# little-little-point-cloud-group/buildingSegment

Measured on AMD Instinct MI355X. Metric: Mpoints/s segmented (kNN+normal+label), higher is better.
Workload: dtype int32 coordinates / f64 normals; 1 GPU; urban_50m; points_per_gpu=50000000, k=16, max_nn=50, rg_mode=0, largest_plane=135921, seed_attempts=6951, fallback_queries=0, rg_rounds=25, validation_rejects=2, tie_rows=971975, parallelism=1 GPU, whole path

## Files before the change

buildingsegment_amd/csrc/bs_knn.hip:

```cpp
#include <algorithm>
#include <cmath>
#include <cstdio>
#include <cstdlib>
#include <type_traits>

#include "bs_common.h"
#include "bs_normal.h"

namespace bs {

namespace {

constexpr int BS_FAST_RINGS = 2;
constexpr int BS_GENERAL_RINGS = 6;

template <bool TILED>
using GridOf = std::conditional_t<TILED, TiledGridDev, GridDev>;

template <bool TILED>
__device__ inline uint64_t cell_key(uint32_t cx, uint32_t cy, uint32_t cz, uint64_t kbase)
{
  if constexpr (TILED)
    return kbase | morton_cell(cx, cy, cz);
  else
    return pack_cell(cx, cy, cz);
}

__device__ inline void tile_enter(TiledGridDev& g, int64_t s, uint64_t& kbase, int64_t& lo, int64_t& hi)
{
  const int32_t t = tile_of(g.tile_off, g.n_tiles, s);
  const TileDesc d = g.tiles[t];
#pragma unroll
  for (int a = 0; a < 3; a++) {
    g.mn[a] = d.mn[a];
    g.dim[a] = d.dim[a];
  }
  kbase = (uint64_t)t << g.mbits;
  lo = g.tile_off[t];
  hi = g.tile_off[t + 1];
}

template <bool TILED = false>
__device__ inline bool cell_lookup(const GridDev& g, uint32_t cx, uint32_t cy, uint32_t cz, int& start,
                                   int& end, uint64_t kbase = 0)
{
  const uint64_t k = cell_key<TILED>(cx, cy, cz, kbase);
  uint32_t h = hash_cell(k) & g.hmask;
  for (;;) {
    const int4 raw = *reinterpret_cast<const int4*>(&g.table[h]);
    const uint64_t ek = (uint64_t)(uint32_t)raw.x | ((uint64_t)(uint32_t)raw.y << 32);
    if (ek == k) {
      start = raw.z;
      end = raw.w;
      return true;
    }
    if (ek == ~0ull)
      return false;
    h = (h + 1) & g.hmask;
  }
}

__device__ inline bool guaranteed_radius(const GridDev& g, const int q[3], const int ci[3], int rho,
                                         uint64_t& R2)
{
  uint32_t R = 0xFFFFFFFFu;
  bool bounded = false;
#pragma unroll
  for (int a = 0; a < 3; a++) {
    if (ci[a] - rho > 0) {
      int lo = g.mn[a] + (ci[a] - rho) * g.cell;
      R = min(R, (uint32_t)(q[a] - lo + 1));
      bounded = true;
    }
    if (ci[a] + rho < g.dim[a] - 1) {
      int hi = g.mn[a] + (ci[a] + rho + 1) * g.cell - 1;
      R = min(R, (uint32_t)(hi + 1 - q[a]));
      bounded = true;
    }
  }
  R2 = (uint64_t)R * (uint64_t)R;
  return bounded;
}

__device__ inline void moments_add(Moments& m, int x, int y, int z)
{
  m.sx += x;
  m.sy += y;
  m.sz += z;
  m.sxx += (uint64_t)((int64_t)x * x);
  m.syy += (uint64_t)((int64_t)y * y);
  m.szz += (uint64_t)((int64_t)z * z);
  m.sxy += (int64_t)x * y;
  m.sxz += (int64_t)x * z;
  m.syz += (int64_t)y * z;
  m.n += 1;
}

template <int KC, bool TILED = false>
__global__ __launch_bounds__(256) void knn_fast_kernel(GridOf<TILED> g, int64_t q_begin, int64_t q_end, int K,
                                                       int max_nn, double r2, int32_t* __restrict__ neigh,
                                                       double* __restrict__ normals,
                                                       int32_t* __restrict__ fb_list,
                                                       int32_t* __restrict__ fb_count, uint64_t cert_r2,
                                                       unsigned long long* __restrict__ uncert,
                                                       int32_t* __restrict__ npos, unsigned long long* __restrict__ tie_rows)
{
  const int64_t s = xcd_logical_block() * (int64_t)blockDim.x + threadIdx.x;
  if (s >= g.n)
    return;
  const int32_t loc = g.slocal[s];
  if (loc < q_begin || loc >= q_end)
    return;
  uint64_t kbase = 0;
  if constexpr (TILED) {
    int64_t lo, hi;
    tile_enter(g, s, kbase, lo, hi);
  }
  uint64_t runner = ~0ull;
  const int4 P = g.spts[s];
  const int q[3] = {P.x, P.y, P.z};
  const int ci[3] = {(int)((uint32_t)(P.x - g.mn[0]) / (uint32_t)g.cell),
                     (int)((uint32_t)(P.y - g.mn[1]) / (uint32_t)g.cell),
                     (int)((uint32_t)(P.z - g.mn[2]) / (uint32_t)g.cell)};
  uint64_t best[KC];
  int bpos[KC];
#pragma unroll
  for (int j = 0; j < KC; j++) {
    best[j] = ~0ull;
    bpos[j] = 0;
  }
  Moments m = {};
  bool done = false;
  for (int rho = 0; rho <= BS_FAST_RINGS && !done; rho++) {
    for (int dz = -rho; dz <= rho; dz++) {
      const int cz = ci[2] + dz;
      if (cz < 0 || cz >= g.dim[2])
        continue;
      for (int dy = -rho; dy <= rho; dy++) {
        const int cy = ci[1] + dy;
        if (cy < 0 || cy >= g.dim[1])
          continue;
        const bool face = (dz == -rho || dz == rho || dy == -rho || dy == rho);
        const int step = face ? 1 : (rho > 0 ? 2 * rho : 1);
        for (int dx = -rho; dx <= rho; dx += step) {
          const int cx = ci[0] + dx;
          if (cx < 0 || cx >= g.dim[0])
            continue;
          int cs, ce;
          if (!cell_lookup<TILED>(g, (uint32_t)cx, (uint32_t)cy, (uint32_t)cz, cs, ce, kbase))
            continue;
          for (int t = cs; t < ce; t++) {
            const int4 c = g.spts[t];
            const int ex = c.x - q[0], ey = c.y - q[1], ez = c.z - q[2];
            const uint32_t d2 = (uint32_t)(ex * ex) + (uint32_t)(ey * ey) + (uint32_t)(ez * ez);
            uint64_t key = ((uint64_t)d2 << 32) | (uint32_t)c.w;
            if (key < best[KC - 1]) {
              int pay = t;
#pragma unroll
              for (int j = 0; j < KC; j++) {
                const bool lt = key < best[j];
                const uint64_t hi = lt ? best[j] : key;
                const int ph = lt ? bpos[j] : pay;
                best[j] = lt ? key : best[j];
                bpos[j] = lt ? pay : bpos[j];
                key = hi;
                pay = ph;
              }
            }
            runner = key < runner ? key : runner;
            if ((double)d2 < r2)
              moments_add(m, c.x, c.y, c.z);
          }
        }
      }
    }
    uint64_t R2;
    const bool bounded = guaranteed_radius(g, q, ci, rho, R2);
    if (!bounded) {
      done = true;
    } else {
      uint64_t kth = ~0ull;
#pragma unroll
      for (int j = 0; j < KC; j++)
        kth = (j == K - 1) ? best[j] : kth;
      const bool knn_ok = kth != ~0ull && (kth >> 32) < R2;
      const bool nrm_ok = (double)R2 >= r2;
      done = knn_ok && nrm_ok;
    }
  }
  uint64_t kth_final = ~0ull;
#pragma unroll
  for (int j = 0; j < KC; j++)
    kth_final = (j == K - 1) ? best[j] : kth_final;
  if (!done || m.n > max_nn || kth_final == ~0ull) {
    const int slot = atomicAdd(fb_count, 1);
    fb_list[slot] = (int32_t)s;
    return;
  }
  int32_t* row = neigh + (int64_t)(loc - q_begin) * K;
#pragma unroll
  for (int j = 0; j < KC; j++)
    if (j < K)
      row[j] = (int32_t)(uint32_t)best[j];
  if (npos) {
    int32_t* prow = npos + s * K;
#pragma unroll
    for (int j = 0; j < KC; j++)
      if (j < K)
        prow[j] = bpos[j];
  }
  if (normals) {
    const V3 nv = normal_from_moments(m);
    double* o = normals + 3 * (int64_t)(loc - q_begin);
    o[0] = nv.x;
    o[1] = nv.y;
    o[2] = nv.z;
    if (npos) {
      double* po = pnorm_of(npos, g.n, K) + 3 * s;
      po[0] = nv.x;
      po[1] = nv.y;
      po[2] = nv.z;
    }
  }
  if (cert_r2 && (kth_final >> 32) >= cert_r2)
    atomicAdd(uncert, 1ull);
  if (tie_rows) {
    bool tie = false;
    uint64_t next = runner;
#pragma unroll
    for (int j = 0; j + 1 < KC; j++) {
      tie = tie || (j + 1 < K && (best[j] >> 32) == (best[j + 1] >> 32));
      next = (j + 1 == K) ? best[j + 1] : next;
    }
    tie = tie || (next != ~0ull && (next >> 32) == (kth_final >> 32));
    if (tie)
      atomicAdd(tie_rows, 1ull);
  }
}

#ifndef BS_KNN_CAP4
#define BS_KNN_CAP4 0
#endif
constexpr int KBUF = 8;
#ifndef BS_KNN_PROBE_GROUP
#define BS_KNN_PROBE_GROUP 3
#endif
#ifdef BS_PROBE
__device__ unsigned long long g_knn_probe[8];
#endif

template <int KC, bool REL32, bool TILED = false, bool STREAM = false>
__global__ __launch_bounds__(256) __attribute__((amdgpu_waves_per_eu(KC == 16 && REL32 && BS_KNN_CAP4 ? 4 : (KC == 16 && REL32 && STREAM ? 3 : 2)))) void knn_fast2_kernel(GridOf<TILED> g, int64_t q_begin, int64_t q_end, int K,
                                                       int max_nn, double r2, uint32_t r2le, int32_t* __restrict__ neigh,
                                                       double* __restrict__ normals,
                                                       int32_t* __restrict__ fb_list,
                                                       int32_t* __restrict__ fb_count, uint64_t cert_r2,
                                                       unsigned long long* __restrict__ uncert,
                                                       int32_t* __restrict__ npos, unsigned long long* __restrict__ tie_rows)
{
  const int64_t s = xcd_logical_block() * (int64_t)blockDim.x + threadIdx.x;
  if (s >= g.n)
    return;
  const int32_t loc = g.slocal[s];
  if (loc < q_begin || loc >= q_end)
    return;
  uint64_t kbase = 0;
  if constexpr (TILED) {
    int64_t lo, hi;
    tile_enter(g, s, kbase, lo, hi);
  }
  uint64_t runner = ~0ull;
  const int4 P = g.spts[s];
  const int q[3] = {P.x, P.y, P.z};
  const int ci[3] = {(int)((uint32_t)(P.x - g.mn[0]) / (uint32_t)g.cell),
                     (int)((uint32_t)(P.y - g.mn[1]) / (uint32_t)g.cell),
                     (int)((uint32_t)(P.z - g.mn[2]) / (uint32_t)g.cell)};
  __shared__ uint32_t blo[KBUF][256], bhi[KBUF][256];
  __shared__ int bps[KBUF][256];
  __shared__ int srs[STREAM ? 9 : 1][STREAM ? 256 : 1], sre[STREAM ? 9 : 1][STREAM ? 256 : 1];
  int nbuf = 0;
  uint64_t best[KC];
  int bpos[KC];
#pragma unroll
  for (int j = 0; j < KC; j++) {
    best[j] = ~0ull;
    bpos[j] = 0;
  }
  Moments m = {};
  int rsx = 0, rsy = 0, rsz = 0, rsxx = 0, rsyy = 0, rszz = 0, rsxy = 0, rsxz = 0, rsyz = 0, rn = 0;
  bool done = false;
  auto flush = [&]() __attribute__((always_inline)) {
    uint64_t bk[KBUF];
    int bp[KBUF];
#pragma unroll
    for (int i = 0; i < KBUF; i++) {
      const bool have = i < nbuf;
      bk[i] = have ? (((uint64_t)bhi[i][threadIdx.x] << 32) | blo[i][threadIdx.x]) : ~0ull;
      bp[i] = have ? bps[i][threadIdx.x] : 0;
    }
    nbuf = 0;
#define BS_CE(ka, pa, kb, pb)            \
  do {                                   \
    const bool sw_ = (kb) < (ka);        \
    const uint64_t tk_ = (ka);           \
    const int tp_ = (pa);                \
    (ka) = sw_ ? (kb) : (ka);            \
    (pa) = sw_ ? (pb) : (pa);            \
    (kb) = sw_ ? tk_ : (kb);             \
    (pb) = sw_ ? tp_ : (pb);             \
  } while (0)
    constexpr int net[19][2] = {{0, 1}, {2, 3}, {4, 5}, {6, 7}, {0, 2}, {1, 3}, {4, 6}, {5, 7}, {1, 2}, {5, 6},
                                {0, 4}, {3, 7}, {1, 5}, {2, 6}, {1, 4}, {3, 6}, {2, 4}, {3, 5}, {3, 4}};
#pragma unroll
    for (int c = 0; c < 19; c++)
      BS_CE(bk[net[c][0]], bp[net[c][0]], bk[net[c][1]], bp[net[c][1]]);
#pragma unroll
    for (int i = 0; i < KBUF; i++)
      BS_CE(best[KC - KBUF + i], bpos[KC - KBUF + i], bk[KBUF - 1 - i], bp[KBUF - 1 - i]);
#pragma unroll
    for (int i = 0; i < KBUF; i++)
      runner = bk[i] < runner ? bk[i] : runner;
#pragma unroll
    for (int d = KC / 2; d >= 1; d >>= 1) {
#pragma unroll
      for (int i = 0; i < KC; i++)
        if ((i & d) == 0)
          BS_CE(best[i], bpos[i], best[i + d], bpos[i + d]);
    }
#undef BS_CE
  };
  auto cand_slot = [&](const int4 c, const int t, const bool real) __attribute__((always_inline)) {
    const int ex = c.x - q[0], ey = c.y - q[1], ez = c.z - q[2];
    const uint32_t d2 = (uint32_t)(ex * ex) + (uint32_t)(ey * ey) + (uint32_t)(ez * ez);
    const uint64_t key = ((uint64_t)d2 << 32) | (uint32_t)c.w;
    if (real && key < best[KC - 1]) {
      blo[nbuf][threadIdx.x] = (uint32_t)key;
      bhi[nbuf][threadIdx.x] = d2;
      bps[nbuf][threadIdx.x] = t;
      nbuf++;
    } else if (real) {
      runner = key < runner ? key : runner;
    }
    if (__ballot(nbuf == KBUF))
      flush();
    if (real && d2 <= r2le) {
      if constexpr (REL32) {
        rsx += ex;
        rsy += ey;
        rsz += ez;
        rsxx += __mul24(ex, ex);
        rsyy += __mul24(ey, ey);
        rszz += __mul24(ez, ez);
        rsxy += __mul24(ex, ey);
        rsxz += __mul24(ex, ez);
        rsyz += __mul24(ey, ez);
        rn += 1;
      } else {
        moments_add(m, c.x, c.y, c.z);
      }
    }
  };
#ifdef BS_PROBE
  int probe_exec = 0, probe_cand = 0;
#define BS_PROBE_BATCH()                                                         \
  do {                                                                           \
    if (rho <= 1 && (int)(threadIdx.x & 63) == __ffsll((long long)__ballot(1)) - 1) \
      probe_exec++;                                                              \
  } while (0)
#define BS_PROBE_CELL(cnt) \
  do {                     \
    if (rho <= 1)          \
      probe_cand += (cnt); \
  } while (0)
#else
#define BS_PROBE_BATCH() \
  do {                   \
  } while (0)
#define BS_PROBE_CELL(cnt) \
  do {                     \
  } while (0)
#endif
  for (int rho = 0; rho <= BS_FAST_RINGS && !done; rho++) {
    const bool streamed = STREAM && rho == 1;
    if (streamed) {
#pragma unroll 1
      for (int dz = -1; dz <= 1; dz++) {
        const int cz = ci[2] + dz;
        const bool zok = cz >= 0 && cz < g.dim[2];
        int cnt = 0;
        constexpr int GP = BS_KNN_PROBE_GROUP;
        static_assert(9 % GP == 0, "probe groups tile the slab");
#pragma unroll
        for (int u0 = 0; u0 < 9; u0 += GP) {
          int4 raw[GP];
          uint64_t ck[GP];
          uint32_t hh[GP];
          bool want[GP];
#pragma unroll
          for (int w = 0; w < GP; w++) {
            const int u = u0 + w;
            const int cy = ci[1] + u / 3 - 1, cx = ci[0] + u % 3 - 1;
            want[w] = zok && cy >= 0 && cy < g.dim[1] && cx >= 0 && cx < g.dim[0] && !(dz == 0 && u == 4);
            ck[w] = cell_key<TILED>((uint32_t)(want[w] ? cx : ci[0]), (uint32_t)(want[w] ? cy : ci[1]),
                                    (uint32_t)(want[w] ? cz : ci[2]), kbase);
            hh[w] = hash_cell(ck[w]) & g.hmask;
            raw[w] = *reinterpret_cast<const int4*>(&g.table[hh[w]]);
          }
#pragma unroll
          for (int w = 0; w < GP; w++) {
            int cs = 0, ce = 0;
            if (want[w]) {
              for (;;) {
                const uint64_t ek = (uint64_t)(uint32_t)raw[w].x | ((uint64_t)(uint32_t)raw[w].y << 32);
                if (ek == ck[w]) {
                  cs = raw[w].z;
                  ce = raw[w].w;
                  break;
                }
                if (ek == ~0ull)
                  break;
                hh[w] = (hh[w] + 1) & g.hmask;
                raw[w] = *reinterpret_cast<const int4*>(&g.table[hh[w]]);
              }
            }
            BS_PROBE_CELL(ce - cs);
            if (cs < ce) {
              srs[cnt][threadIdx.x] = cs;
              sre[cnt][threadIdx.x] = ce;
              cnt++;
            }
          }
        }
        int cur = 0;
        int t0 = cnt > 0 ? srs[0][threadIdx.x] : 0, e0 = cnt > 0 ? sre[0][threadIdx.x] : 0;
        int s1 = cnt > 1 ? srs[1][threadIdx.x] : 0, e1 = cnt > 1 ? sre[1][threadIdx.x] : 0;
        while (t0 < e0) {
          BS_PROBE_BATCH();
          const int rem = e0 - t0;
          int ta[4];
          bool rl[4];
          int4 cc[4];
#pragma unroll
          for (int v = 0; v < 4; v++) {
            const int t1 = s1 + (v - rem);
            rl[v] = v < rem || t1 < e1;
            ta[v] = v < rem ? t0 + v : t1;
            cc[v] = g.spts[rl[v] ? ta[v] : (int)s];
          }
#pragma unroll
          for (int v = 0; v < 4; v++)
            cand_slot(cc[v], ta[v], rl[v]);
          const bool pop1 = rem <= 4;
          t0 += pop1 ? 0 : 4;
          if (__ballot(pop1)) {
            const bool more1 = pop1 && cur + 2 < cnt;
            const int i2 = min(cur + 2, 8);
            const int s2 = more1 ? srs[i2][threadIdx.x] : 0, e2 = more1 ? sre[i2][threadIdx.x] : 0;
            t0 = pop1 ? s1 + (4 - rem) : t0;
            e0 = pop1 ? e1 : e0;
            s1 = pop1 ? s2 : s1;
            e1 = pop1 ? e2 : e1;
            cur += pop1 ? 1 : 0;
            const bool pop2 = pop1 && e0 != 0 && t0 >= e0;
            if (__ballot(pop2)) {
              const bool more2 = pop2 && cur + 2 < cnt;
              const int i3 = min(cur + 2, 8);
              const int s3 = more2 ? srs[i3][threadIdx.x] : 0, e3 = more2 ? sre[i3][threadIdx.x] : 0;
              t0 = pop2 ? s1 : t0;
              e0 = pop2 ? e1 : e0;
              s1 = pop2 ? s3 : s1;
              e1 = pop2 ? e3 : e1;
              cur += pop2 ? 1 : 0;
            }
          }
        }
      }
    }
    for (int dz = -rho; !streamed && dz <= rho; dz++) {
      const int cz = ci[2] + dz;
      if (cz < 0 || cz >= g.dim[2])
        continue;
      for (int dy = -rho; dy <= rho; dy++) {
        const int cy = ci[1] + dy;
        if (cy < 0 || cy >= g.dim[1])
          continue;
        const bool face = (dz == -rho || dz == rho || dy == -rho || dy == rho);
        const int step = face ? 1 : (rho > 0 ? 2 * rho : 1);
        for (int dx0 = -rho; dx0 <= rho; dx0 += 3 * step) {
          int4 raw[3];
          uint64_t ck[3];
          uint32_t hh[3];
          bool want[3];
#pragma unroll
          for (int u = 0; u < 3; u++) {
            const int dx = dx0 + u * step;
            const int cx = ci[0] + dx;
            want[u] = dx <= rho && cx >= 0 && cx < g.dim[0];
            ck[u] = cell_key<TILED>((uint32_t)(want[u] ? cx : ci[0]), (uint32_t)cy, (uint32_t)cz, kbase);
            hh[u] = hash_cell(ck[u]) & g.hmask;
            raw[u] = *reinterpret_cast<const int4*>(&g.table[hh[u]]);
          }
          int cs3[3], ce3[3];
#pragma unroll
          for (int u = 0; u < 3; u++) {
            cs3[u] = 0;
            ce3[u] = 0;
            if (!want[u])
              continue;
            for (;;) {
              const uint64_t ek = (uint64_t)(uint32_t)raw[u].x | ((uint64_t)(uint32_t)raw[u].y << 32);
              if (ek == ck[u]) {
                cs3[u] = raw[u].z;
                ce3[u] = raw[u].w;
                break;
              }
              if (ek == ~0ull)
                break;
              hh[u] = (hh[u] + 1) & g.hmask;
              raw[u] = *reinterpret_cast<const int4*>(&g.table[hh[u]]);
            }
          }
#pragma unroll 1
          for (int u = 0; u < 3; u++) {
            const int cs = u == 0 ? cs3[0] : (u == 1 ? cs3[1] : cs3[2]);
            const int ce = u == 0 ? ce3[0] : (u == 1 ? ce3[1] : ce3[2]);
            BS_PROBE_CELL(ce - cs);
            for (int t0 = cs; t0 < ce; t0 += 4) {
              BS_PROBE_BATCH();
              int4 cc[4];
#pragma unroll
              for (int v = 0; v < 4; v++)
                cc[v] = g.spts[t0 + v < ce ? t0 + v : ce - 1];
#pragma unroll
              for (int v = 0; v < 4; v++)
                cand_slot(cc[v], t0 + v, t0 + v < ce);
            }
          }
        }
      }
    }
    if (__ballot(nbuf > 0))
      flush();
    uint64_t R2;
    const bool bounded = guaranteed_radius(g, q, ci, rho, R2);
    if (!bounded) {
      done = true;
    } else {
      uint64_t kth = ~0ull;
#pragma unroll
      for (int j = 0; j < KC; j++)
        kth = (j == K - 1) ? best[j] : kth;
      const bool knn_ok = kth != ~0ull && (kth >> 32) < R2;
      const bool nrm_ok = (double)R2 >= r2;
      done = knn_ok && nrm_ok;
    }
  }
#undef BS_PROBE_BATCH
#undef BS_PROBE_CELL
#ifdef BS_PROBE
  {
    const unsigned long long act = __ballot(1);
    const int lane = threadIdx.x & 63;
    const int need = (probe_cand + 3) / 4;
    int ex_sum = probe_exec, nd_max = need, nd_sum = need, ln = 1;
    for (int o = 32; o > 0; o >>= 1) {
      const int a = __shfl_xor(ex_sum, o), b = __shfl_xor(nd_max, o), c = __shfl_xor(nd_sum, o), d = __shfl_xor(ln, o);
      const bool ok = (act >> (lane ^ o)) & 1;
      ex_sum += ok ? a : 0;
      nd_max = ok && b > nd_max ? b : nd_max;
      nd_sum += ok ? c : 0;
      ln += ok ? d : 0;
    }
    if (lane == __ffsll((long long)act) - 1) {
      atomicAdd(&g_knn_probe[0], (unsigned long long)ex_sum);
      atomicAdd(&g_knn_probe[1], (unsigned long long)nd_max);
      atomicAdd(&g_knn_probe[2], (unsigned long long)nd_sum);
      atomicAdd(&g_knn_probe[3], (unsigned long long)ln);
      atomicAdd(&g_knn_probe[4], 1ull);
    }
  }
#endif
  uint64_t kth_final = ~0ull;
#pragma unroll
  for (int j = 0; j < KC; j++)
    kth_final = (j == K - 1) ? best[j] : kth_final;
  if constexpr (REL32) {
    const int64_t n64 = rn, qx = q[0], qy = q[1], qz = q[2];
    m.n = rn;
    m.sx = n64 * qx + rsx;
    m.sy = n64 * qy + rsy;
    m.sz = n64 * qz + rsz;
    m.sxx = (uint64_t)(n64 * qx * qx + 2 * qx * rsx + rsxx);
    m.syy = (uint64_t)(n64 * qy * qy + 2 * qy * rsy + rsyy);
    m.szz = (uint64_t)(n64 * qz * qz + 2 * qz * rsz + rszz);
    m.sxy = n64 * qx * qy + qx * rsy + qy * rsx + rsxy;
    m.sxz = n64 * qx * qz + qx * rsz + qz * rsx + rsxz;
    m.syz = n64 * qy * qz + qy * rsz + qz * rsy + rsyz;
  }
  if (!done || m.n > max_nn || kth_final == ~0ull) {
    const int slot = atomicAdd(fb_count, 1);
    fb_list[slot] = (int32_t)s;
    return;
  }
  int32_t* row = neigh + (int64_t)(loc - q_begin) * K;
#pragma unroll
  for (int j = 0; j < KC; j++)
    if (j < K)
      row[j] = (int32_t)(uint32_t)best[j];
  if (npos) {
    int32_t* prow = npos + s * K;
#pragma unroll
    for (int j = 0; j < KC; j++)
      if (j < K)
        prow[j] = bpos[j];
  }
  if (normals) {
    const V3 nv = normal_from_moments(m);
    double* o = normals + 3 * (int64_t)(loc - q_begin);
    o[0] = nv.x;
    o[1] = nv.y;
    o[2] = nv.z;
    if (npos) {
      double* po = pnorm_of(npos, g.n, K) + 3 * s;
      po[0] = nv.x;
      po[1] = nv.y;
      po[2] = nv.z;
    }
  }
  if (cert_r2 && (kth_final >> 32) >= cert_r2)
    atomicAdd(uncert, 1ull);
  if (tie_rows) {
    bool tie = false;
    uint64_t next = runner;
#pragma unroll
    for (int j = 0; j + 1 < KC; j++) {
      tie = tie || (j + 1 < K && (best[j] >> 32) == (best[j + 1] >> 32));
      next = (j + 1 == K) ? best[j + 1] : next;
    }
    tie = tie || (next != ~0ull && (next >> 32) == (kth_final >> 32));
    if (tie)
      atomicAdd(tie_rows, 1ull);
  }
}


__device__ inline bool cand_less(uint64_t d2a, int32_t ia, uint64_t d2b, int32_t ib)
{
  return d2a < d2b || (d2a == d2b && ia < ib);
}

__device__ inline void list_insert(uint64_t* d2s, int32_t* idxs, int32_t* poss, int& cnt, int cap, uint64_t d2, int32_t idx,
                                   int32_t pos, uint64_t* out_d2 = nullptr)
{
  int c = cnt;
  if (c == cap) {
    if (!cand_less(d2, idx, d2s[cap - 1], idxs[cap - 1])) {
      if (out_d2 && d2 < *out_d2)
        *out_d2 = d2;
      return;
    }
    if (out_d2 && d2s[cap - 1] < *out_d2)
      *out_d2 = d2s[cap - 1];
    c = cap - 1;
  }
  int j = c;
  while (j > 0 && cand_less(d2, idx, d2s[j - 1], idxs[j - 1])) {
    d2s[j] = d2s[j - 1];
    idxs[j] = idxs[j - 1];
    poss[j] = poss[j - 1];
    j--;
  }
  d2s[j] = d2;
  idxs[j] = idx;
  poss[j] = pos;
  cnt = c + 1;
}

__device__ inline void hybrid_insert(uint64_t* d2s, int32_t* gids, int32_t* poss, int& cnt, int cap,
                                     uint64_t d2, int32_t gid, int32_t pos)
{
  int c = cnt;
  if (c == cap) {
    if (!cand_less(d2, gid, d2s[cap - 1], gids[cap - 1]))
      return;
    c = cap - 1;
  }
  int j = c;
  while (j > 0 && cand_less(d2, gid, d2s[j - 1], gids[j - 1])) {
    d2s[j] = d2s[j - 1];
    gids[j] = gids[j - 1];
    poss[j] = poss[j - 1];
    j--;
  }
  d2s[j] = d2;
  gids[j] = gid;
  poss[j] = pos;
  cnt = c + 1;
}

template <bool TILED = false>
__global__ __launch_bounds__(64) void knn_general_kernel(GridOf<TILED> g, int64_t q_begin, int K, int max_nn,
                                                         double r2, int32_t* __restrict__ neigh,
                                                         double* __restrict__ normals,
                                                         const int32_t* __restrict__ fb_list,
                                                         const int32_t* __restrict__ fb_count,
                                                         uint64_t cert_r2,
                                                         unsigned long long* __restrict__ uncert,
                                                         int32_t* __restrict__ npos, unsigned long long* __restrict__ tie_rows)
{
  const int total = *fb_count;
  for (int w = blockIdx.x * blockDim.x + threadIdx.x; w < total; w += gridDim.x * blockDim.x) {
    const int32_t s = fb_list[w];
    const int32_t loc = g.slocal[s];
    uint64_t kbase = 0;
    int64_t scan_lo = 0, scan_hi = g.n;
    if constexpr (TILED)
      tile_enter(g, s, kbase, scan_lo, scan_hi);
    const int4 P = g.spts[s];
    const int q[3] = {P.x, P.y, P.z};
    const int ci[3] = {(int)((uint32_t)(P.x - g.mn[0]) / (uint32_t)g.cell),
                       (int)((uint32_t)(P.y - g.mn[1]) / (uint32_t)g.cell),
                       (int)((uint32_t)(P.z - g.mn[2]) / (uint32_t)g.cell)};
    uint64_t kd2[32], md2[64];
    int32_t kidx[32], kpos[32], mgid[64], mpos[64];
    int kc = 0, mc = 0;
    uint64_t runner = ~0ull;
    bool done = false;
    for (int rho = 0; rho <= BS_GENERAL_RINGS && !done; rho++) {
      for (int dz = -rho; dz <= rho; dz++) {
        const int cz = ci[2] + dz;
        if (cz < 0 || cz >= g.dim[2])
          continue;
        for (int dy = -rho; dy <= rho; dy++) {
          const int cy = ci[1] + dy;
          if (cy < 0 || cy >= g.dim[1])
            continue;
          const bool face = (dz == -rho || dz == rho || dy == -rho || dy == rho);
          const int step = face ? 1 : (rho > 0 ? 2 * rho : 1);
          for (int dx = -rho; dx <= rho; dx += step) {
            const int cx = ci[0] + dx;
            if (cx < 0 || cx >= g.dim[0])
              continue;
            int cs, ce;
            if (!cell_lookup<TILED>(g, (uint32_t)cx, (uint32_t)cy, (uint32_t)cz, cs, ce, kbase))
              continue;
            for (int t = cs; t < ce; t++) {
              const int4 c = g.spts[t];
              const int64_t ex = (int64_t)c.x - q[0], ey = (int64_t)c.y - q[1], ez = (int64_t)c.z - q[2];
              const uint64_t d2 = (uint64_t)(ex * ex) + (uint64_t)(ey * ey) + (uint64_t)(ez * ez);
              list_insert(kd2, kidx, kpos, kc, K, d2, c.w, t, &runner);
              if ((double)d2 < r2)
                hybrid_insert(md2, mgid, mpos, mc, max_nn, d2, c.w, t);
            }
          }
        }
      }
      uint64_t R2;
      const bool bounded = guaranteed_radius(g, q, ci, rho, R2);
      if (!bounded)
        done = true;
      else
        done = (kc == K) && (kd2[K - 1] < R2) && ((double)R2 >= r2);
    }
    if (!done) {
      kc = 0;
      mc = 0;
      runner = ~0ull;
      for (int64_t t = scan_lo; t < scan_hi; t++) {
        const int4 c = g.spts[t];
        const int64_t ex = (int64_t)c.x - q[0], ey = (int64_t)c.y - q[1], ez = (int64_t)c.z - q[2];
        const uint64_t d2 = (uint64_t)(ex * ex) + (uint64_t)(ey * ey) + (uint64_t)(ez * ez);
        list_insert(kd2, kidx, kpos, kc, K, d2, c.w, (int32_t)t, &runner);
        if ((double)d2 < r2)
          hybrid_insert(md2, mgid, mpos, mc, max_nn, d2, c.w, (int32_t)t);
      }
    }
    int32_t* row = neigh + (int64_t)(loc - q_begin) * K;
    for (int j = 0; j < K; j++)
      row[j] = kidx[j];
    if (npos)
      for (int j = 0; j < K; j++)
        npos[(int64_t)s * K + j] = kpos[j];
    if (normals) {
      Moments m = {};
      for (int j = 0; j < mc; j++) {
        const int4 c = g.spts[mpos[j]];
        moments_add(m, c.x, c.y, c.z);
      }
      const V3 nv = normal_from_moments(m);
      double* o = normals + 3 * (int64_t)(loc - q_begin);
      o[0] = nv.x;
      o[1] = nv.y;
      o[2] = nv.z;
      if (npos) {
        double* po = pnorm_of(npos, g.n, K) + 3 * (int64_t)s;
        po[0] = nv.x;
        po[1] = nv.y;
        po[2] = nv.z;
      }
    }
    if (cert_r2 && kd2[K - 1] >= cert_r2)
      atomicAdd(uncert, 1ull);
    if (tie_rows) {
      bool tie = runner == kd2[K - 1];
      for (int j = 0; j + 1 < K; j++)
        tie = tie || kd2[j] == kd2[j + 1];
      if (tie)
        atomicAdd(tie_rows, 1ull);
    }
  }
}

constexpr int GCAP = 2048;

template <bool TILED = false>
__global__ __launch_bounds__(64) void knn_general_wave_kernel(GridOf<TILED> g, int64_t q_begin, int K, int max_nn, double r2,
                                                              int32_t* __restrict__ neigh, double* __restrict__ normals,
                                                              const int32_t* __restrict__ fb_list,
                                                              const int32_t* __restrict__ fb_count, uint64_t cert_r2,
                                                              unsigned long long* __restrict__ uncert,
                                                              int32_t* __restrict__ npos, unsigned long long* __restrict__ tie_rows,
                                                              int32_t* __restrict__ fb2_list, int32_t* __restrict__ fb2_count)
{
  __shared__ uint64_t bd2[GCAP];
  __shared__ int32_t bidx[GCAP], bpos[GCAP];
  __shared__ int cxyz[64][3];
  const int lane = threadIdx.x;
  const int total = *fb_count;
  for (int w = blockIdx.x; w < total; w += gridDim.x) {
    const int32_t s = fb_list[w];
    const int32_t loc = g.slocal[s];
    uint64_t kbase = 0;
    if constexpr (TILED) {
      int64_t lo, hi;
      tile_enter(g, s, kbase, lo, hi);
    }
    const int4 P = g.spts[s];
    const int q[3] = {P.x, P.y, P.z};
    const int ci[3] = {(int)((uint32_t)(P.x - g.mn[0]) / (uint32_t)g.cell),
                       (int)((uint32_t)(P.y - g.mn[1]) / (uint32_t)g.cell),
                       (int)((uint32_t)(P.z - g.mn[2]) / (uint32_t)g.cell)};
    int count = 0;
    bool done = false, overflow = false;
    for (int rho = 0; rho <= BS_GENERAL_RINGS && !done && !overflow; rho++) {
      const int side = 2 * rho + 1, ncell = side * side * side;
      for (int c0 = 0; c0 < ncell; c0 += 64) {
        const int c = c0 + lane;
        const int dz = c / (side * side) - rho, dy = (c / side) % side - rho, dx = c % side - rho;
        const int cx = ci[0] + dx, cy = ci[1] + dy, cz = ci[2] + dz;
        const int cheb = max(max(abs(dx), abs(dy)), abs(dz));
        int cs = 0, ce = 0;
        if (c < ncell && cheb == rho && cx >= 0 && cx < g.dim[0] && cy >= 0 && cy < g.dim[1] && cz >= 0 && cz < g.dim[2]) {
          if (!cell_lookup<TILED>(g, (uint32_t)cx, (uint32_t)cy, (uint32_t)cz, cs, ce, kbase))
            cs = ce = 0;
        }
        for (int t = cs; __ballot(t < ce) != 0; t++) {
          const bool have = t < ce;
          const unsigned long long m = __ballot(have);
          const int slot = count + __popcll(m & ((1ull << lane) - 1ull));
          if (have && slot < GCAP) {
            const int4 p = g.spts[t];
            const int64_t ex = (int64_t)p.x - q[0], ey = (int64_t)p.y - q[1], ez = (int64_t)p.z - q[2];
            bd2[slot] = (uint64_t)(ex * ex) + (uint64_t)(ey * ey) + (uint64_t)(ez * ez);
            bidx[slot] = p.w;
            bpos[slot] = t;
          }
          count += __popcll(m);
        }
      }
      if (count > GCAP) {
        overflow = true;
        break;
      }
      int P2 = 64;
      while (P2 < count)
        P2 <<= 1;
      for (int i = count + lane; i < P2; i += 64) {
        bd2[i] = ~0ull;
        bidx[i] = 0x7fffffff;
        bpos[i] = 0;
      }
      __syncthreads();
      for (int k2 = 2; k2 <= P2; k2 <<= 1) {
        for (int j = k2 >> 1; j > 0; j >>= 1) {
          for (int i = lane; i < P2; i += 64) {
            const int l = i ^ j;
            if (l > i) {
              const uint64_t da = bd2[i], db = bd2[l];
              const int32_t ia = bidx[i], ib = bidx[l];
              const bool a_gt_b = da > db || (da == db && ia > ib);
              const bool up = (i & k2) == 0;
              if (a_gt_b == up) {
                bd2[i] = db;
                bd2[l] = da;
                bidx[i] = ib;
                bidx[l] = ia;
                const int32_t pa = bpos[i];
                bpos[i] = bpos[l];
                bpos[l] = pa;
              }
            }
          }
          __syncthreads();
        }
      }
      uint64_t R2;
      const bool bounded = guaranteed_radius(g, q, ci, rho, R2);
      if (!bounded)
        done = true;
      else
        done = count >= K && bd2[K - 1] < R2 && (double)R2 >= r2;
      __syncthreads();
    }
    if (overflow || !done || count < K) {
      if (lane == 0)
        fb2_list[atomicAdd(fb2_count, 1)] = s;
      __syncthreads();
      continue;
    }
    if (lane < K) {
      neigh[(int64_t)(loc - q_begin) * K + lane] = bidx[lane];
      if (npos)
        npos[(int64_t)s * K + lane] = bpos[lane];
    }
    if (normals) {
      const bool in = lane < max_nn && lane < count && (double)bd2[lane] < r2;
      const int mc = __popcll(__ballot(in));
      if (in) {
        const int4 p = g.spts[bpos[lane]];
        cxyz[lane][0] = p.x;
        cxyz[lane][1] = p.y;
        cxyz[lane][2] = p.z;
      }
      __syncthreads();
      if (lane == 0) {
        Moments m = {};
        for (int j = 0; j < mc; j++)
          moments_add(m, cxyz[j][0], cxyz[j][1], cxyz[j][2]);
        const V3 nv = normal_from_moments(m);
        double* o = normals + 3 * (int64_t)(loc - q_begin);
        o[0] = nv.x;
        o[1] = nv.y;
        o[2] = nv.z;
        if (npos) {
          double* po = pnorm_of(npos, g.n, K) + 3 * (int64_t)s;
          po[0] = nv.x;
          po[1] = nv.y;
          po[2] = nv.z;
        }
      }
    }
    if (lane == 0) {
      if (cert_r2 && bd2[K - 1] >= cert_r2)
        atomicAdd(uncert, 1ull);
      if (tie_rows) {
        bool tie = count > K && bd2[K] == bd2[K - 1];
        for (int j = 0; j + 1 < K; j++)
          tie = tie || bd2[j] == bd2[j + 1];
        if (tie)
          atomicAdd(tie_rows, 1ull);
      }
    }
    __syncthreads();
  }
}

__global__ void mark_all_kernel(GridDev g, int64_t q_begin, int64_t q_end, int32_t* fb_list,
                                int32_t* fb_count)
{
  const int64_t s = blockIdx.x * (int64_t)blockDim.x + threadIdx.x;
  if (s >= g.n)
    return;
  const int32_t loc = g.slocal[s];
  if (loc < q_begin || loc >= q_end)
    return;
  fb_list[atomicAdd(fb_count, 1)] = (int32_t)s;
}

}

template <bool TILED>
static int launch_knn(bs_ctx* ctx, const GridOf<TILED>& g, int64_t q_begin, int64_t q_end, const bs_params& p,
                      int32_t* d_neigh, double* d_normals, double cert_radius, int64_t* n_uncertified, int32_t* d_npos)
{
  hipStream_t st = ctx->stream;
  const int64_t n = g.n;
  BS_HIP(ctx, ctx->fb_list.reserve(sizeof(int32_t) * (2 * n + 32)));
  int32_t* fb_list = ctx->fb_list.as<int32_t>() + 16;
  int32_t* fb_count = ctx->fb_list.as<int32_t>();
  int32_t* fb2_list = fb_list + n + 16;
  int32_t* fb2_count = ctx->fb_list.as<int32_t>() + 2;
  unsigned long long* uncert = (unsigned long long*)(ctx->fb_list.as<int32_t>() + 4);
  unsigned long long* tie_rows = (unsigned long long*)(ctx->fb_list.as<int32_t>() + 8);
  BS_HIP(ctx, hipMemsetAsync(ctx->fb_list.p, 0, 64, st));
  const double r2 = p.radius * p.radius;
  uint64_t cert_r2 = 0;
  if (cert_radius > 0) {
    double c2 = cert_radius * cert_radius;
    cert_r2 = c2 >= 1.8e19 ? ~0ull : (uint64_t)std::ceil(c2);
    if (cert_r2 == 0)
      cert_r2 = 1;
  }
  const int blocks = (int)((n + 255) / 256);
  const int xblocks = xcd_grid(blocks);
  const bool fast_ok = (int64_t)g.cell * (2 * BS_FAST_RINGS + 1) <= 37500;
  if (fast_ok) {
    const bool buffered = getenv("BS_KNN_BUFFERED") ? atoi(getenv("BS_KNN_BUFFERED")) != 0 : true;
    const bool rel32 = r2 <= 32761.0 && !getenv("BS_KNN_MOMENTS64");
    const bool stream = (getenv("BS_KNN_STREAM") ? atoi(getenv("BS_KNN_STREAM")) != 0 : true) && !(TILED && p.k <= 16 && !rel32);
    const uint32_t r2le = (uint32_t)(std::min(std::ceil(r2), 4294967296.0) - 1.0);
#define BS_FAST2(KC_, REL_)                                                                                              \
  do {                                                                                                                   \
    if (stream)                                                                                                          \
      knn_fast2_kernel<KC_, REL_, TILED, true><<<xblocks, 256, 0, st>>>(g, q_begin, q_end, p.k, p.max_nn, r2, r2le, d_neigh, \
                                                                        d_normals, fb_list, fb_count, cert_r2, uncert,  \
                                                                        d_npos, tie_rows);                              \
    else                                                                                                                 \
      knn_fast2_kernel<KC_, REL_, TILED, false><<<xblocks, 256, 0, st>>>(g, q_begin, q_end, p.k, p.max_nn, r2, r2le, d_neigh, \
                                                                         d_normals, fb_list, fb_count, cert_r2, uncert, \
                                                                         d_npos, tie_rows);                             \
  } while (0)
    if (buffered && p.k <= 16 && rel32)
      BS_FAST2(16, true);
    else if (buffered && p.k <= 16)
      BS_FAST2(16, false);
    else if (buffered && rel32)
      BS_FAST2(32, true);
    else if (buffered)
      BS_FAST2(32, false);
#undef BS_FAST2
    else if (p.k <= 16)
      knn_fast_kernel<16, TILED><<<xblocks, 256, 0, st>>>(g, q_begin, q_end, p.k, p.max_nn, r2, d_neigh, d_normals,
                                                  fb_list, fb_count, cert_r2, uncert, d_npos, tie_rows);
    else
      knn_fast_kernel<32, TILED><<<xblocks, 256, 0, st>>>(g, q_begin, q_end, p.k, p.max_nn, r2, d_neigh, d_normals,
                                                  fb_list, fb_count, cert_r2, uncert, d_npos, tie_rows);
  } else {
    mark_all_kernel<<<blocks, 256, 0, st>>>(g, q_begin, q_end, fb_list, fb_count);
  }
  if (getenv("BS_KNN_GENERAL_THREAD")) {
    knn_general_kernel<TILED><<<1024, 64, 0, st>>>(g, q_begin, p.k, p.max_nn, r2, d_neigh, d_normals, fb_list, fb_count, cert_r2,
                                            uncert, d_npos, tie_rows);
  } else {
    knn_general_wave_kernel<TILED><<<8192, 64, 0, st>>>(g, q_begin, p.k, p.max_nn, r2, d_neigh, d_normals, fb_list, fb_count, cert_r2,
                                                 uncert, d_npos, tie_rows, fb2_list, fb2_count);
    knn_general_kernel<TILED><<<1024, 64, 0, st>>>(g, q_begin, p.k, p.max_nn, r2, d_neigh, d_normals, fb2_list, fb2_count, cert_r2,
                                            uncert, d_npos, tie_rows);
  }
  BS_HIP(ctx, hipGetLastError());
  int32_t hb[4];
  BS_HIP(ctx, hipMemcpyAsync(hb, ctx->fb_list.p, sizeof hb, hipMemcpyDeviceToHost, st));
  unsigned long long hu = 0, ht = 0;
  BS_HIP(ctx, hipMemcpyAsync(&hu, uncert, sizeof hu, hipMemcpyDeviceToHost, st));
  BS_HIP(ctx, hipMemcpyAsync(&ht, tie_rows, sizeof ht, hipMemcpyDeviceToHost, st));
  BS_HIP(ctx, hipStreamSynchronize(st));
#ifdef BS_PROBE
  {
    unsigned long long pr[8] = {};
    BS_HIP(ctx, hipMemcpyFromSymbol(pr, HIP_SYMBOL(g_knn_probe), sizeof pr));
    if (pr[4])
      fprintf(stderr, "knn probe: waves %llu lanes %llu executed batches/wave %.2f largest need/wave %.2f mean need/lane %.2f "
                      "executed/largest %.3f\n", pr[4], pr[3], (double)pr[0] / pr[4], (double)pr[1] / pr[4],
              (double)pr[2] / pr[3], (double)pr[0] / (double)pr[1]);
    const unsigned long long zero[8] = {};
    BS_HIP(ctx, hipMemcpyToSymbol(HIP_SYMBOL(g_knn_probe), zero, sizeof zero));
  }
#endif
  ctx->tm.n_fallback_queries = hb[0];
  ctx->tm.tie_rows = (int64_t)ht;
  if (n_uncertified)
    *n_uncertified = (int64_t)hu;
  return BS_OK;
}

int launch_knn_normals(bs_ctx* ctx, const GridDev& g, int64_t q_begin, int64_t q_end, const bs_params& p,
                       int32_t* d_neigh, double* d_normals, double cert_radius, int64_t* n_uncertified, int32_t* d_npos)
{
  return launch_knn<false>(ctx, g, q_begin, q_end, p, d_neigh, d_normals, cert_radius, n_uncertified, d_npos);
}

int launch_knn_normals_tiled(bs_ctx* ctx, const TiledGridDev& g, const bs_params& p, int32_t* d_neigh,
                             double* d_normals, int32_t* d_npos)
{
  return launch_knn<true>(ctx, g, 0, g.n, p, d_neigh, d_normals, 0.0, nullptr, d_npos);
}

}
```

Measured before the change: 201.0 Mpoints/s.

## Cap kNN admissions by the ring-1 guaranteed radius and defer the ring-0 flush

For k<=16 on large clouds, the fast kNN kernel seeds an admission bound from the guaranteed radius of ring 1. Candidates at or beyond that radius skip the shared-memory buffer and the sorting-network flush. The end-of-ring-0 flush is skipped unless some lane has already seen K candidates. If the cap leaves the result unfinished, the kernel reruns rings 0-1 with the cap removed and without accumulating normal moments a second time. This trades fewer flushes and admissions against extra register state and a possible second pass. It also adds more detailed probe counters.

```diff
diff --git a/buildingsegment_amd/csrc/bs_knn.hip b/buildingsegment_amd/csrc/bs_knn.hip
--- a/buildingsegment_amd/csrc/bs_knn.hip
+++ b/buildingsegment_amd/csrc/bs_knn.hip
@@ -246,7 +246,7 @@
 #define BS_KNN_PROBE_GROUP 3
 #endif
 #ifdef BS_PROBE
-__device__ unsigned long long g_knn_probe[8];
+__device__ unsigned long long g_knn_probe[24];
 #endif
 
 template <int KC, bool REL32, bool TILED = false, bool STREAM = false>
@@ -256,7 +256,8 @@
                                                        int32_t* __restrict__ fb_list,
                                                        int32_t* __restrict__ fb_count, uint64_t cert_r2,
                                                        unsigned long long* __restrict__ uncert,
-                                                       int32_t* __restrict__ npos, unsigned long long* __restrict__ tie_rows)
+                                                       int32_t* __restrict__ npos, unsigned long long* __restrict__ tie_rows,
+                                                       int cap_on)
 {
   const int64_t s = xcd_logical_block() * (int64_t)blockDim.x + threadIdx.x;
   if (s >= g.n)
@@ -289,7 +290,43 @@
   Moments m = {};
   int rsx = 0, rsy = 0, rsz = 0, rsxx = 0, rsyy = 0, rszz = 0, rsxy = 0, rsxz = 0, rsyz = 0, rn = 0;
   bool done = false;
+  uint64_t capkey = ~0ull;
+  if (cap_on) {
+    uint64_t R2_1;
+    if (guaranteed_radius(g, q, ci, 1, R2_1) && R2_1 < (1ull << 32))
+      capkey = R2_1 << 32;
+  }
+  uint64_t bound = capkey;
+  int seen0 = 0;
+  bool ball_on = true;
+#ifdef BS_PROBE
+  int probe_flush = 0, probe_flush01 = 0, probe_adm = 0, probe_far = 0, probe_seen0 = 0;
+  int probe_r0flush = 0, probe_r0nodone = 0, probe_r0nok = 0, probe_ring2 = 0;
+  bool probe_r01 = true, probe_r0 = true;
+  uint64_t probe_R2 = ~0ull;
+  if (!guaranteed_radius(g, q, ci, 1, probe_R2))
+    probe_R2 = ~0ull;
+#define BS_PROBE_FLUSH()              \
+  do {                                \
+    probe_flush++;                    \
+    probe_flush01 += probe_r01 ? 1 : 0; \
+  } while (0)
+#define BS_PROBE_SLOT(real_, adm_, d2_)                                  \
+  do {                                                                   \
+    probe_seen0 += (real_) && probe_r0 ? 1 : 0;                          \
+    probe_adm += (adm_) && probe_r01 ? 1 : 0;                            \
+    probe_far += (adm_) && probe_r01 && (uint64_t)(d2_) >= probe_R2 ? 1 : 0; \
+  } while (0)
+#else
+#define BS_PROBE_FLUSH() \
+  do {                   \
+  } while (0)
+#define BS_PROBE_SLOT(real_, adm_, d2_) \
+  do {                                  \
+  } while (0)
+#endif
   auto flush = [&]() __attribute__((always_inline)) {
+    BS_PROBE_FLUSH();
     uint64_t bk[KBUF];
     int bp[KBUF];
 #pragma unroll
@@ -328,12 +365,14 @@
           BS_CE(best[i], bpos[i], best[i + d], bpos[i + d]);
     }
 #undef BS_CE
+    bound = best[KC - 1] < capkey ? best[KC - 1] : capkey;
   };
   auto cand_slot = [&](const int4 c, const int t, const bool real) __attribute__((always_inline)) {
     const int ex = c.x - q[0], ey = c.y - q[1], ez = c.z - q[2];
     const uint32_t d2 = (uint32_t)(ex * ex) + (uint32_t)(ey * ey) + (uint32_t)(ez * ez);
     const uint64_t key = ((uint64_t)d2 << 32) | (uint32_t)c.w;
-    if (real && key < best[KC - 1]) {
+    BS_PROBE_SLOT(real, real && key < bound, d2);
+    if (real && key < bound) {
       blo[nbuf][threadIdx.x] = (uint32_t)key;
       bhi[nbuf][threadIdx.x] = d2;
       bps[nbuf][threadIdx.x] = t;
@@ -343,7 +382,7 @@
     }
     if (__ballot(nbuf == KBUF))
       flush();
-    if (real && d2 <= r2le) {
+    if (real && ball_on && d2 <= r2le) {
       if constexpr (REL32) {
         rsx += ex;
         rsy += ey;
@@ -364,12 +403,12 @@
   int probe_exec = 0, probe_cand = 0;
 #define BS_PROBE_BATCH()                                                         \
   do {                                                                           \
-    if (rho <= 1 && (int)(threadIdx.x & 63) == __ffsll((long long)__ballot(1)) - 1) \
+    if (probe_r01 && (int)(threadIdx.x & 63) == __ffsll((long long)__ballot(1)) - 1) \
       probe_exec++;                                                              \
   } while (0)
 #define BS_PROBE_CELL(cnt) \
   do {                     \
-    if (rho <= 1)          \
+    if (probe_r01)         \
       probe_cand += (cnt); \
   } while (0)
 #else
@@ -380,7 +419,26 @@
   do {                     \
   } while (0)
 #endif
-  for (int rho = 0; rho <= BS_FAST_RINGS && !done; rho++) {
+  const int nstep = BS_FAST_RINGS + 1 + (cap_on ? 2 : 0);
+  for (int step = 0; step < nstep && !done; step++) {
+    const bool again = cap_on && step >= 2;
+    const int rho = again ? step - 2 : step;
+    if (again && rho == 0) {
+#pragma unroll
+      for (int j = 0; j < KC; j++) {
+        best[j] = ~0ull;
+        bpos[j] = 0;
+      }
+      runner = ~0ull;
+      capkey = ~0ull;
+      bound = ~0ull;
+      seen0 = 0;
+    }
+    ball_on = !(again && rho <= 1);
+#ifdef BS_PROBE
+    probe_r01 = !again && rho <= 1;
+    probe_r0 = !again && rho == 0;
+#endif
     const bool streamed = STREAM && rho == 1;
     if (streamed) {
 #pragma unroll 1
@@ -525,6 +583,8 @@
             const int cs = u == 0 ? cs3[0] : (u == 1 ? cs3[1] : cs3[2]);
             const int ce = u == 0 ? ce3[0] : (u == 1 ? ce3[1] : ce3[2]);
             BS_PROBE_CELL(ce - cs);
+            if (rho == 0)
+              seen0 += ce - cs;
             for (int t0 = cs; t0 < ce; t0 += 4) {
               BS_PROBE_BATCH();
               int4 cc[4];
@@ -539,8 +599,13 @@
         }
       }
     }
-    if (__ballot(nbuf > 0))
+#ifdef BS_PROBE
+    const bool probe_endflush = __ballot(nbuf > 0) != 0;
+#endif
+    if ((rho != 0 || __ballot(seen0 >= K)) && __ballot(nbuf > 0))
       flush();
+    if (again && rho <= 1)
+      continue;
     uint64_t R2;
     const bool bounded = guaranteed_radius(g, q, ci, rho, R2);
     if (!bounded) {
@@ -554,7 +619,18 @@
       const bool nrm_ok = (double)R2 >= r2;
       done = knn_ok && nrm_ok;
     }
-  }
+#ifdef BS_PROBE
+    if (probe_r0) {
+      probe_r0flush = probe_endflush ? 1 : 0;
+      probe_r0nodone = probe_endflush && __ballot(done) == 0 ? 1 : 0;
+      probe_r0nok = probe_endflush && __ballot(probe_seen0 >= K) == 0 ? 1 : 0;
+    }
+    if (probe_r01 && rho == 1)
+      probe_ring2 = done ? 0 : 1;
+#endif
+  }
+#undef BS_PROBE_FLUSH
+#undef BS_PROBE_SLOT
 #undef BS_PROBE_BATCH
 #undef BS_PROBE_CELL
 #ifdef BS_PROBE
@@ -563,6 +639,9 @@
     const int lane = threadIdx.x & 63;
     const int need = (probe_cand + 3) / 4;
     int ex_sum = probe_exec, nd_max = need, nd_sum = need, ln = 1;
+    int mx[8] = {probe_flush, probe_flush01, probe_adm, probe_adm - probe_far, probe_r0flush, probe_r0nodone, probe_r0nok,
+                 probe_ring2};
+    int sm[3] = {probe_adm, probe_far, probe_ring2};
     for (int o = 32; o > 0; o >>= 1) {
       const int a = __shfl_xor(ex_sum, o), b = __shfl_xor(nd_max, o), c = __shfl_xor(nd_sum, o), d = __shfl_xor(ln, o);
       const bool ok = (act >> (lane ^ o)) & 1;
@@ -570,6 +649,16 @@
       nd_max = ok && b > nd_max ? b : nd_max;
       nd_sum += ok ? c : 0;
       ln += ok ? d : 0;
+#pragma unroll
+      for (int i = 0; i < 8; i++) {
+        const int v = __shfl_xor(mx[i], o);
+        mx[i] = ok && v > mx[i] ? v : mx[i];
+      }
+#pragma unroll
+      for (int i = 0; i < 3; i++) {
+        const int v = __shfl_xor(sm[i], o);
+        sm[i] += ok ? v : 0;
+      }
     }
     if (lane == __ffsll((long long)act) - 1) {
       atomicAdd(&g_knn_probe[0], (unsigned long long)ex_sum);
@@ -577,6 +666,12 @@
       atomicAdd(&g_knn_probe[2], (unsigned long long)nd_sum);
       atomicAdd(&g_knn_probe[3], (unsigned long long)ln);
       atomicAdd(&g_knn_probe[4], 1ull);
+#pragma unroll
+      for (int i = 0; i < 8; i++)
+        atomicAdd(&g_knn_probe[5 + i], (unsigned long long)mx[i]);
+#pragma unroll
+      for (int i = 0; i < 3; i++)
+        atomicAdd(&g_knn_probe[13 + i], (unsigned long long)sm[i]);
     }
   }
 #endif
@@ -1008,17 +1103,19 @@
     const bool buffered = getenv("BS_KNN_BUFFERED") ? atoi(getenv("BS_KNN_BUFFERED")) != 0 : true;
     const bool rel32 = r2 <= 32761.0 && !getenv("BS_KNN_MOMENTS64");
     const bool stream = (getenv("BS_KNN_STREAM") ? atoi(getenv("BS_KNN_STREAM")) != 0 : true) && !(TILED && p.k <= 16 && !rel32);
+    const char* cap_env = getenv("BS_KNN_CAP");
+    const int cap = cap_env ? (atoi(cap_env) != 0) : (p.k <= 16 && n >= ((int64_t)1 << 23));
     const uint32_t r2le = (uint32_t)(std::min(std::ceil(r2), 4294967296.0) - 1.0);
 #define BS_FAST2(KC_, REL_)                                                                                              \
   do {                                                                                                                   \
     if (stream)                                                                                                          \
       knn_fast2_kernel<KC_, REL_, TILED, true><<<xblocks, 256, 0, st>>>(g, q_begin, q_end, p.k, p.max_nn, r2, r2le, d_neigh, \
                                                                         d_normals, fb_list, fb_count, cert_r2, uncert,  \
-                                                                        d_npos, tie_rows);                              \
+                                                                        d_npos, tie_rows, cap);                         \
     else                                                                                                                 \
       knn_fast2_kernel<KC_, REL_, TILED, false><<<xblocks, 256, 0, st>>>(g, q_begin, q_end, p.k, p.max_nn, r2, r2le, d_neigh, \
                                                                          d_normals, fb_list, fb_count, cert_r2, uncert, \
-                                                                         d_npos, tie_rows);                             \
+                                                                         d_npos, tie_rows, cap);                        \
   } while (0)
     if (buffered && p.k <= 16 && rel32)
       BS_FAST2(16, true);
@@ -1056,13 +1153,21 @@
   BS_HIP(ctx, hipStreamSynchronize(st));
 #ifdef BS_PROBE
   {
-    unsigned long long pr[8] = {};
+    unsigned long long pr[24] = {};
     BS_HIP(ctx, hipMemcpyFromSymbol(pr, HIP_SYMBOL(g_knn_probe), sizeof pr));
-    if (pr[4])
+    if (pr[4]) {
+      const double w = (double)pr[4], l = (double)pr[3];
       fprintf(stderr, "knn probe: waves %llu lanes %llu executed batches/wave %.2f largest need/wave %.2f mean need/lane %.2f "
                       "executed/largest %.3f\n", pr[4], pr[3], (double)pr[0] / pr[4], (double)pr[1] / pr[4],
               (double)pr[2] / pr[3], (double)pr[0] / (double)pr[1]);
-    const unsigned long long zero[8] = {};
+      fprintf(stderr, "knn probe: per wave: flushes %.3f (rings 0-1: %.3f), admissions of the fullest lane %.2f, without those "
+                      "at or beyond R2(1) %.2f, waves with candidates waiting at the end of ring 0 %.3f, no lane done "
+                      "there %.3f, no lane had seen K %.3f\n",
+              pr[5] / w, pr[6] / w, pr[7] / w, pr[8] / w, pr[9] / w, pr[10] / w, pr[11] / w);
+      fprintf(stderr, "knn probe: per lane: admissions %.2f, at or beyond R2(1) %.2f; lanes going on to ring 2 %.5f of all, "
+                      "waves holding one %.5f of all\n", pr[13] / l, pr[14] / l, pr[15] / l, pr[12] / w);
+    }
+    const unsigned long long zero[24] = {};
     BS_HIP(ctx, hipMemcpyToSymbol(HIP_SYMBOL(g_knn_probe), zero, sizeof zero));
   }
 #endif
```

After: 201.5 Mpoints/s, median of 4. About the same (+0.2%).
